# Borx25/CPU-Raytracing-experiments

Hardware: AMD Instinct MI355X
Metric: Mray/s (primary+bounce) (higher is better)
Workload: dtype f32; 1 GPU; cfg4: 4096x4096 px, S(100000) spheres + SAH BVH, MIS, Policy.max_bounces=9 (primary+8 bounces), 5 buckets, 64 accumulations/step; fixed image, tile rows split over the GPUs; image=4096x4096, spheres=100000, max_bounces=9, buckets=5, parallelism=single GPU, batches_in_flight=1, accumulations_per_batch=63, accumulations_per_batch_limit=63

## Files before the change

cpu-raytracing-experiments_amd/__init__.py:

```python
from __future__ import annotations

import ctypes as C
import os
import subprocess

import numpy as np

from . import distributed as distributed
from . import hdr as hdr
from . import scene as scene
from .scene import MATERIAL, NODE, SPHERE, Camera, Scene

_HERE = os.path.dirname(os.path.abspath(__file__))
CSRC = os.path.join(_HERE, "csrc")
LIB_PATH = os.path.join(CSRC, "libmirt.so")

MIRT_OK, MIRT_NOT_READY = 0, 1
AOV_DEPTH, AOV_NORMAL, AOV_ALBEDO = 0, 1, 2
AOV_PLANES = 7
KERNEL_CLASSES = ("raygen", "trace", "shade", "shadow", "resolve")


class MirtError(RuntimeError):
    pass
# ... 64 lines not shown
        "mirt_aov_floats": [P, C.POINTER(C.c_size_t)],
        "mirt_read_aov": [P, vp],
        "mirt_aov_device": [P, C.POINTER(vp), C.POINTER(C.c_size_t)],
        "mirt_load_aov": [P, vp, i32],
        "mirt_render_aov": [P, i32, vp],
        "mirt_get_counters": [P, C.POINTER(Counters)],
        "mirt_get_kernel_times": [P, C.POINTER(KernelTimes), i32],
        "mirt_get_stream": [P, C.POINTER(vp)],
        "mirt_debug_raygen": [P, u32, vp, vp],
        "mirt_debug_trace_closest": [P, C.c_size_t, vp, vp, vp, vp],
        "mirt_debug_trace_shadow": [P, C.c_size_t, vp, vp, vp, vp],
        "mirt_debug_math": [P, i32, C.c_size_t, vp, vp],
        "mirt_debug_info": [P, vp],
        "mirt_debug_tree": [P, vp, C.c_size_t, vp],
        "mirt_debug_primary_lists": [P, vp],
        "mirt_debug_allow_half_boxes": [P, i32],
    }
    G = C.c_void_p
    sigs.update({
        "mirt_group_create": [vp, i32, C.POINTER(G)],
        "mirt_group_destroy": [G],
        "mirt_group_size": [G, C.POINTER(i32)],
        "mirt_group_member": [G, i32, C.POINTER(P)],
        "mirt_group_set_scene": [G, vp, vp, u32, vp, u32, vp, u32, vp, u32, vp, vp, u32, u32],
        "mirt_group_set_camera": [G, vp, vp, f, f, f, f],
        "mirt_group_set_lens": [G, f, f],
        "mirt_group_pick_focus": [G, u32, u32, C.POINTER(f), C.POINTER(f)],
        "mirt_group_set_policy": [G, C.POINTER(Policy)],
        "mirt_group_set_gloss_decay": [G, vp, u32],
        "mirt_group_set_stream_order": [G, u32],
# ... 290 lines not shown
        return d

    def debug_tree(self):
        info = (C.c_uint32 * 4)()
        self._check(self._lib.mirt_debug_tree(self._ctx, None, 0, info))
        n, rec_bytes = int(info[0]), int(info[1])
        words = np.zeros((n, rec_bytes // 4), dtype=np.uint32)
        self._check(self._lib.mirt_debug_tree(self._ctx, _ptr(words), words.nbytes, info))
        return words, dict(zip(("records", "record_bytes", "layout", "depth"), [int(v) for v in info]))

    def debug_primary_lists(self) -> list:
        out = (C.c_uint32 * 10)()
        self._check(self._lib.mirt_debug_primary_lists(self._ctx, out))
        return [int(v) for v in out]

    def stream_handle(self) -> int:
        p = C.c_void_p()
        self._check(self._lib.mirt_get_stream(self._ctx, C.byref(p)))
        return p.value

    def debug_raygen(self, accumulations: int):
        n = (self.width // 16) * (self.height // 16) * 256
        p = np.empty((3, n), dtype=np.float32)
        d = np.empty((3, n), dtype=np.float32)
        self._check(self._lib.mirt_debug_raygen(self._ctx, accumulations, _ptr(p), _ptr(d)))
        return p, d

    def debug_trace_closest(self, p: np.ndarray, d: np.ndarray):
        p = np.ascontiguousarray(p, dtype=np.float32); d = np.ascontiguousarray(d, dtype=np.float32)
        n = p.shape[1]
# ... 189 lines not shown
```

cpu-raytracing-experiments_amd/csrc/kernels.hpp:

```cpp
#pragma once
#include <hip/hip_runtime.h>
#include <stdint.h>
#include "device_math.hpp"

namespace mirt {

constexpr uint32_t kBlock = 256;
constexpr uint32_t kShadeBlock = 512;
constexpr uint32_t kTraceBlock = 1024;
constexpr uint32_t kLdsStack = 16;
constexpr uint32_t kLdsStackWide = 12;
constexpr uint32_t kLeafBit = 0x80000000u;
constexpr uint32_t kTileSize = 256;
constexpr uint32_t kTileRoot = 16;
constexpr uint32_t kStack = 64;
constexpr uint32_t kDestAccum = 0x80000000u;

struct SceneDev {
	const float4* recs;
	const float4* spheres;
	const int32_t* prim_mat;
	const float4* light_sphere;
	const float4* light_emit;
	const float4* mat_albedo;
// ... 242 lines not shown
	float px, py, pz, dx, dy, dz;
	RaySlab rs;
	float tfar;
	int32_t prim;
	uint32_t cur, sp;
};
struct TravSpill { uint32_t e[kStack - kLdsStackWide]; };
constexpr float kAlphaFat = 0.03f;
MIRT_DI bool trav_begin(Trav& t, float px, float py, float pz, float dx, float dy, float dz, float tfar, float alpha_extra = 0.0f) {
	t.px = px; t.py = py; t.pz = pz; t.dx = dx; t.dy = dy; t.dz = dz;
	float alpha;
	t.rs = make_slab(px, py, pz, dx, dy, dz, alpha, alpha_extra);
	t.tfar = tfar; t.prim = -1; t.cur = 0; t.sp = 0;
	return alpha > kAlphaFat;
}
constexpr int kClosest = 0, kAnyHit = 1, kCollect = 2;
constexpr uint32_t kCandMax = 31, kCandStride = 32, kCandOverflow = 0xffffffffu;
struct Collect { uint32_t* cand; float rho; uint32_t n_pix; };
MIRT_DI void collect_leaf(bool on, float4 s, uint32_t prim, uint32_t pix, const Collect& col, Trav& t) {
	uint32_t cnt = static_cast<uint32_t>(t.prim);
	if (on & (cnt < kCandMax)) col.cand[static_cast<size_t>(1u + cnt) * col.n_pix + pix] = prim;
	cnt += on ? 1u : 0u;
	t.prim = static_cast<int32_t>(cnt);
	const f3 oc{ s.x - t.px, s.y - t.py, s.z - t.pz };
	const float oc2 = dot3(oc, oc), b = dot3(f3{ t.dx, t.dy, t.dz }, oc);
	const float len = __builtin_sqrtf(oc2);
	const float reach = __builtin_sqrtf(__builtin_fmaxf(oc2 - b * b, 0.0f)) + col.rho * len;
	const float slack = (s.w - reach * reach) - (0x1p-17f * oc2 + 1e-6f * s.w);
	const bool cover = on & (b > 0.0f) & (oc2 > s.w * 1.002f) & (slack > 0.0f);
	const float F = ((b + col.rho * len) - __builtin_sqrtf(__builtin_fmaxf(slack, 0.0f))) * 1.001f + 1e-4f;
	t.tfar = (cover & (F < t.tfar)) ? F : t.tfar;
}
typedef __attribute__((address_space(3))) int16_t lds_i16;
template <bool HALF, bool ST16>
MIRT_DI void stack_put(const TraceLds lds, TravSpill& spill, uint32_t sp, uint32_t ref) {
	constexpr uint32_t lds_entries = (HALF && !ST16) ? kLdsStackWide : kLdsStack;
// ... 109 lines not shown
		if (hd && (!cd || !d_cd)) { stack_put<true, ST16>(lds, spill, sp, r3); sp += 1u; }
	}
	uint32_t next = any ? near : kHalt;
	if (!any & (sp != 0u)) { --sp; next = stack_get<true, ST16>(lds, spill, sp); }
	t.sp = sp;
	t.cur = next;
}
template <int MODE, bool COUNT, bool ALL_LDS, bool HALF, bool ST16>
MIRT_DI void leaf_step(const SceneDev& sc, const TraceLds lds, Trav& t, TravSpill& spill, bool& occluded, uint32_t& n_spheres, uint32_t pix, const Collect& col) {
	const uint32_t first = t.cur & ~kLeafBit;
	float4 s;
	if (ALL_LDS) s = to_float4(lds.spheres[first]); else s = sc.spheres[first];
	if (COUNT) n_spheres += 1u;
	bool fin = false;
	if (MODE == kAnyHit) { occluded = sphere_occludes_sel(s, t.px, t.py, t.pz, t.dx, t.dy, t.dz, t.tfar); fin = occluded; }
	else if (MODE == kCollect) { collect_leaf(true, s, first, pix, col, t); fin = static_cast<uint32_t>(t.prim) > kCandMax; }
	else sphere_closest_sel(true, s, static_cast<int32_t>(first), t.px, t.py, t.pz, t.dx, t.dy, t.dz, t.tfar, t.prim);
	uint32_t sp = t.sp;
	t.cur = kHalt;
	if (!fin & (sp != 0u)) { --sp; t.cur = stack_get<HALF, ST16>(lds, spill, sp); }
	t.sp = sp;
}

constexpr uint32_t kChunkMax = 512;
constexpr uint32_t kLeafBatch = 16;
constexpr uint32_t kRefillIdle = 32;
constexpr uint32_t kNone = 0xffffffffu;
struct FatList { uint32_t* count; uint32_t* rays; uint32_t capacity; };
struct WaveWindow { uint32_t beg, end, chunk_end, offset, chunk; bool more; };
MIRT_DI uint32_t pick_chunk(uint32_t n, uint32_t chunk_max) {
	const uint32_t waves = gridDim.x * (blockDim.x >> 6);
// ... 30 lines not shown
                              LoadRay load_ray, StoreResult store_result, const Collect col = Collect{ nullptr, 0.0f, 0u }) {
	WaveWindow w{ 0, 0, 0, 0, pick_chunk(n, sc.chunk_max), true };
	Trav t;
	TravSpill spill;
	uint32_t ri = kNone;
	bool occluded = false;
	t.cur = kHalt;
	for (;;) {
		if ((ri != kNone) & (t.cur == kHalt)) { store_result(ri, t, occluded); ri = kNone; }
		{
			const uint32_t got = wave_take(ri == kNone, w, q, n, work_next);
			if (got != kNone) {
				float px, py, pz, dx, dy, dz, tf;
				load_ray(got, px, py, pz, dx, dy, dz, tf);
				ri = got; occluded = false;
				if (MODE == kCollect) {
					if (trav_begin(t, px, py, pz, dx, dy, dz, tf, col.rho)) { t.prim = static_cast<int32_t>(kCandMax + 1u); t.cur = kHalt; }
					else t.prim = 0;
				} else if (trav_begin(t, px, py, pz, dx, dy, dz, tf)) {
					const uint32_t k = atomicAdd(fat.count, 1u);
					if (k < fat.capacity) { fat.rays[k] = got; ri = kNone; t.cur = kHalt; }
				}
			}
		}
		const bool work_left = w.more || w.beg != w.chunk_end;
		if (__ballot(ri != kNone) == 0ull) { if (!work_left) break; continue; }
		const bool can_refill = work_left;
		for (;;) {
			const bool at_leaf = static_cast<int32_t>(t.cur) < 0, at_node = t.cur < kHalt;
			const unsigned long long leaf_m = __ballot(at_leaf), node_m = __ballot(at_node);
			const unsigned long long walking = leaf_m | node_m;
			if (walking == 0ull) break;
// ... 342 lines not shown
			float tfar = MIRT_FLT_MAX; int32_t prim = -1;
			for (uint32_t k = 0; k < kCandRegs; k++) if (id[k] >= 0) sphere_closest_tie(s[k], id[k], ox, oy, oz, d.x, d.y, d.z, tfar, prim);
			for (uint32_t k = kCandRegs; k < kCandMax; k++) {
				if (__ballot(k < cnt) == 0ull) break;
				if (k < cnt) {
					const uint32_t j = cand[static_cast<size_t>(k + 1u) * fp.n_pix + pix];
					sphere_closest_tie(sc.spheres[j], static_cast<int32_t>(j), ox, oy, oz, d.x, d.y, d.z, tfar, prim);
				}
			}
			if (COUNT) c_spheres += cnt;
			const size_t i = static_cast<size_t>(slot) * fp.n_pix + pix;
			hit_out[i] = HitRec{ tfar, prim };
		}
	}
	if (COUNT) wave_sum(c_spheres, &ctr->spheres);
}

constexpr uint32_t kAovPlanes = 7;
constexpr float kAovMissDepth = 1e4f;
template <bool LENS = false>
__global__ __launch_bounds__(kBlock) void k_first_hit_aov(SceneDev sc, FrameParams fp, const HitRec* __restrict__ hit_in, const float4* __restrict__ mat_colour, float* __restrict__ aov, LensParams lens) {
	f3 O{ fp.cam.pos[0], fp.cam.pos[1], fp.cam.pos[2] };
	for (uint32_t pix = blockIdx.x * kBlock + threadIdx.x; pix < fp.n_pix; pix += gridDim.x * kBlock) {
		uint32_t tile; int32_t x, y;
		pixel_xy(fp, pix, tile, x, y);
		const uint32_t seed = (tile * kTileSize + (pix & 255u)) * (fp.max_bounces * 2u + 1u);
		float* w = aov + static_cast<size_t>(pix >> 8) * (kAovPlanes * kTileSize) + (pix & 255u);
		float sum[kAovPlanes];
		for (uint32_t k = 0; k < kAovPlanes; k++) sum[k] = w[k * kTileSize];
		int32_t cached = -1;
// ... 660 lines not shown
```

cpu-raytracing-experiments_amd/csrc/mirt_capi.hip:

```cpp
#include "../../include/mirt.h"
#include "kernels.hpp"
#include "bvh_layout.hpp"
#include "bvh_build.hpp"
#include "lbvh_build.hpp"

#include <hip/hip_runtime.h>
#include <algorithm>
#include <cstdarg>
#include <cstdio>
#include <cstdlib>
#include <cstring>
#include <string>
#include <vector>

using namespace mirt;

namespace {

thread_local std::string g_create_error;

struct DeviceBuffer {
	void* ptr = nullptr;
	size_t bytes = 0;
	hipError_t ensure(size_t want) {
// ... 51 lines not shown
	DeviceBuffer recs, recs_wide, spheres, prim_mat, light_sphere, light_emit, mat_albedo, mat_emission, mat_ggx, hdri;
	SceneDev scene{};
	std::vector<float> gloss_decay;
	uint32_t stream_order = 0;
	DeviceBuffer gloss_decay_dev;
	bool gloss_decay_dev_valid = false;
	CameraParams camera{};
	LensParams lens{};
	uint32_t bvh_depth = 0;
	DeviceBuffer cand;
	DeviceBuffer cand_listed;
	DeviceBuffer cand_words;
	hipEvent_t cand_built = nullptr;
	uint64_t cand_gen = 0;
	bool cand_valid = false;
	bool allow_half = true;

	DeviceBuffer accumulator;
	uint32_t aov_on = 0;
	DeviceBuffer aov;
	hipEvent_t aov_prev = nullptr;
	DeviceBuffer framebuffer;
	float* frame_host = nullptr;
	size_t frame_host_bytes = 0;
	DeviceBuffer counters;
	std::vector<PipeSlot> slots;
	uint64_t planned_for = 0;
	uint32_t batch_mem_cap = 256;
	uint32_t capacity = 0;
	uint32_t seg_cap = 0;
// ... 85 lines not shown
struct BatchCounters {
	uint32_t* w; uint32_t nb, seg_cap;
	static size_t words(uint32_t nb) { return static_cast<size_t>(2 * nb + 2) * kQueueWords + static_cast<size_t>(nb) * 4 + 8; }
	Queue queue(uint32_t k) const { return Queue{ w + static_cast<size_t>(k) * kQueueWords, seg_cap }; }
	uint32_t* word(uint32_t k) const { return w + static_cast<size_t>(2 * nb + 2) * kQueueWords + k; }
	Queue stream_queue(uint32_t b) const { return queue(b); }
	Queue shadow_queue(uint32_t b) const { return queue(nb + 1 + b); }
	Queue empty_queue() const { return queue(2 * nb + 1); }
	uint32_t* closest_work(uint32_t b) const { return word(b); }
	uint32_t* shadow_work(uint32_t b) const { return word(nb + b); }
	FatList fat_closest(uint32_t b, uint32_t* lists) const { return FatList{ word(2 * nb + b), lists, kFatCapacity }; }
	FatList fat_shadow(uint32_t b, uint32_t* lists) const { return FatList{ word(3 * nb + b), lists + kFatCapacity, kFatCapacity }; }
};
struct CandWords {
	uint32_t* w;
	static constexpr size_t kWords = 4;
	uint32_t* work() const { return w; }
	uint32_t* unused_fat_count() const { return w + 1; }
	uint32_t* listed_pixels() const { return w + 2; }
};
BatchCounters batch_counters(const mirt_ctx* c, const PipeSlot& sl) { return BatchCounters{ sl.counts.as<uint32_t>(), c->policy.max_bounces, c->seg_cap }; }
uint32_t wanted_slots(const mirt_ctx* c) {
	if (c->policy.streams) return std::min<uint32_t>(c->policy.streams, 8u);
	return static_cast<uint64_t>(c->n_tiles) * kTileSize * batch_limit(c) >= kSerialRays ? 1u : 3u;
}
uint64_t streams_bytes(const mirt_ctx* c) {
	const uint64_t rays = static_cast<uint64_t>(c->n_tiles) * kTileSize * batch_limit(c);
	return wanted_slots(c) * (rays * 4u * kStreamPlanes + rays * 12u);
}

void plan_batches(mirt_ctx* c) {
	const uint64_t n_pix = static_cast<uint64_t>(c->n_tiles) * kTileSize;
	if (c->policy.max_batch || n_pix == 0 || c->planned_for == n_pix) return;
	c->batch_mem_cap = kMaxBatch;
// ... 165 lines not shown

const decltype(&k_trace<true, kPrimaryNone>) kTrace[2][3] = {
	{ k_trace<true, kPrimaryNone>, k_trace<true, kPrimaryAll>, k_trace<true, kPrimaryList> },
	{ k_trace<false, kPrimaryNone>, k_trace<false, kPrimaryAll>, k_trace<false, kPrimaryList> } };
const decltype(&k_trace_fat<true, kPrimaryNone>) kTraceFat[2][3] = {
	{ k_trace_fat<true, kPrimaryNone>, k_trace_fat<true, kPrimaryAll>, k_trace_fat<true, kPrimaryList> },
	{ k_trace_fat<false, kPrimaryNone>, k_trace_fat<false, kPrimaryAll>, k_trace_fat<false, kPrimaryList> } };
const decltype(&k_primary_cand<true>) kPrimaryCand[2] = { k_primary_cand<true>, k_primary_cand<false> };
const decltype(&k_primary_hits<true>) kPrimaryHits[2] = { k_primary_hits<true>, k_primary_hits<false> };
const decltype(&k_shade<false, false>) kShade[2][2] = { { k_shade<false, false>, k_shade<false, true> }, { k_shade<true, false>, k_shade<true, true> } };
const decltype(&k_tile_stream<false>) kTileStream[2] = { k_tile_stream<false>, k_tile_stream<true> };
static_assert(kPrimaryNone == 0 && kPrimaryAll == 1 && kPrimaryList == 2, "kTrace / kTraceFat are indexed by PRIMARY");
const decltype(&k_trace<true, kPrimaryNone>) kTraceLens[2] = { k_trace<true, kPrimaryAll, true>, k_trace<false, kPrimaryAll, true> };
const decltype(&k_trace_fat<true, kPrimaryNone>) kTraceFatLens[2] = { k_trace_fat<true, kPrimaryAll, true>, k_trace_fat<false, kPrimaryAll, true> };
const decltype(&k_shade<false, false>) kShadeLens[2] = { k_shade<true, false, true>, k_shade<true, true, true> };

struct TraceLaunch {
	StreamBuf in; HitRec* hit;
	Queue closest_queue; uint32_t* closest_work;
	ShadowBuf sh; ShadowSink sink;
	Queue shadow_queue; uint32_t* shadow_work;
	FatList fat_closest, fat_shadow;
	const uint32_t* listed_pixels;
	DevCounters* ctr;
};
void launch_trace(const mirt_ctx* c, hipStream_t st, const SceneDev& sc, const FrameParams& fp, uint64_t n_rays, bool count, int primary, const TraceLaunch& t, bool lens = false) {
	hipLaunchKernelGGL(lens ? kTraceLens[!count] : kTrace[!count][primary], dim3(trace_grid(c, n_rays)), dim3(kTraceBlock), trace_lds(c), st, sc, fp, t.in, t.hit, t.closest_queue, t.closest_work,
	                   t.sh, t.sink, t.shadow_queue, t.shadow_work, t.fat_closest, t.fat_shadow, t.ctr, c->lens);
	const uint32_t fat_grid = sc.n_spheres > 4096 ? static_cast<uint32_t>(c->n_cu) * 2u : 64u;
	if (sc.use_bvh) hipLaunchKernelGGL(lens ? kTraceFatLens[!count] : kTraceFat[!count][primary], dim3(fat_grid), dim3(1024), 0, st, sc, fp, t.in, t.hit, t.fat_closest, t.sh, t.sink, t.fat_shadow, t.ctr, t.listed_pixels, c->lens);
}

int launch_tile_stream(mirt_ctx* c, hipStream_t st, const SceneDev& sc, const FrameParams& fp, uint32_t batch_n, float* contrib, DevCounters* ctr, bool count) {
	if (!c->gloss_decay_dev_valid) {
		HIP_TRY(c, sync_all(c));
		HIP_TRY(c, c->gloss_decay_dev.ensure(std::max<size_t>(c->gloss_decay.size(), 1) * sizeof(float)));
		if (!c->gloss_decay.empty()) HIP_TRY(c, hipMemcpy(c->gloss_decay_dev.ptr, c->gloss_decay.data(), c->gloss_decay.size() * sizeof(float), hipMemcpyHostToDevice));
		c->gloss_decay_dev_valid = true;
	}
	Bracket t(c, MIRT_K_TRACE, st);
	hipLaunchKernelGGL(kTileStream[c->policy.brdf != 0], dim3(c->n_tiles * batch_n), dim3(kTileSize), 0, st, sc, fp, contrib, ctr, c->mat_ggx.as<float4>(),
	                   c->gloss_decay_dev.as<float>(), static_cast<uint32_t>(c->gloss_decay.size()), count ? 1u : 0u);
	return MIRT_OK;
}

int build_primary_lists(mirt_ctx* c, const SceneDev& sc, const FrameParams& fp, bool count) {
	HIP_TRY(c, c->cand.ensure(static_cast<size_t>(fp.n_pix) * kCandStride * sizeof(uint32_t)));
	HIP_TRY(c, c->cand_listed.ensure(static_cast<size_t>(fp.n_pix) * sizeof(uint32_t)));
	HIP_TRY(c, c->cand_words.ensure(CandWords::kWords * sizeof(uint32_t)));
	if (!c->cand_built) HIP_TRY(c, hipEventCreateWithFlags(&c->cand_built, hipEventDisableTiming));
	const CandWords cw{ c->cand_words.as<uint32_t>() };
	HIP_TRY(c, hipMemsetAsync(cw.w, 0, CandWords::kWords * sizeof(uint32_t), c->stream));
	{ Bracket t(c, MIRT_K_TRACE);
	  const FatList none{ cw.unused_fat_count(), nullptr, 0u };
	  hipLaunchKernelGGL(kPrimaryCand[!count], dim3(trace_grid(c, fp.n_pix)), dim3(kTraceBlock), trace_lds(c), c->stream, sc, fp, c->cand.as<uint32_t>(), bundle_half_angle(c),
	                     cw.work(), none, c->counters.as<DevCounters>(), c->cand_listed.as<uint32_t>(), cw.listed_pixels()); }
	HIP_TRY(c, hipGetLastError());
	HIP_TRY(c, hipEventRecord(c->cand_built, c->stream));
	c->cand_gen++;
	c->cand_valid = true;
	return MIRT_OK;
}

int launch_first_hit_aov(mirt_ctx* c, PipeSlot& sl, hipStream_t st, const SceneDev& sc, const FrameParams& fp) {
	const bool pipelined = c->slots.size() > 1;
	if (pipelined) {
		if (!sl.aov_done) HIP_TRY(c, hipEventCreateWithFlags(&sl.aov_done, hipEventDisableTiming));
		if (c->aov_prev && c->aov_prev != sl.aov_done) HIP_TRY(c, hipStreamWaitEvent(st, c->aov_prev, 0));
	}
	{ Bracket t(c, MIRT_K_RESOLVE, st);
	  const uint32_t grid = static_cast<uint32_t>(std::min<uint64_t>((static_cast<uint64_t>(fp.n_pix) + kBlock - 1) / kBlock, static_cast<uint64_t>(c->n_cu) * 64u));
	  hipLaunchKernelGGL(lens_on(c) ? k_first_hit_aov<true> : k_first_hit_aov<false>, dim3(grid), dim3(kBlock), 0, st, sc, fp, sl.hit, c->policy.brdf ? c->mat_ggx.as<float4>() : c->scene.mat_albedo,
// ... 21 lines not shown
	const SceneDev sc = trace_scene(c);
	const bool count = c->policy.count_traffic != 0;
	const uint32_t sgrid = static_cast<uint32_t>(std::min<uint64_t>((total + kShadeBlock - 1) / kShadeBlock, static_cast<uint64_t>(c->n_cu) * c->tune_shade_wgs));
	{
		const uint64_t n_chunks = (static_cast<uint64_t>(fp.n_pix) + kShadeBlock - 1) / kShadeBlock;
		const uint64_t want = (8ull * sgrid + n_chunks - 1) / n_chunks;
		fp.first_groups = static_cast<uint32_t>(std::min<uint64_t>(std::max<uint64_t>(want, 1), batch_n));
	}

	if (pipelined && sl.in_use) HIP_TRY(c, hipStreamWaitEvent(st, sl.merged, 0));
	if (c->debug_poison_contrib)
		HIP_TRY(c, hipMemsetD32Async(reinterpret_cast<hipDeviceptr_t>(sl.contrib.ptr), 0x7fc0deadu, sl.contrib.bytes / sizeof(float), st));
	HIP_TRY(c, hipMemsetAsync(bc.w, 0, BatchCounters::words(nb) * sizeof(uint32_t), st));
	if (bundle) {
		if (!c->cand_valid || count) { const int r = build_primary_lists(c, sc, fp, count); if (r) return r; }
		if (pipelined && sl.cand_gen != c->cand_gen) { HIP_TRY(c, hipStreamWaitEvent(st, c->cand_built, 0)); sl.cand_gen = c->cand_gen; }
	}
	const CandWords cw{ c->cand_words.as<uint32_t>() };
	if (c->stream_order) {
		const int r = launch_tile_stream(c, st, sc, fp, batch_n, contrib, ctr, count);
		if (r) return r;
	} else {
		for (uint32_t bounce = 0; bounce < nb; bounce++) {
			const StreamBuf& in = sl.stream_buf[bounce & 1u];
			const StreamBuf& out = sl.stream_buf[(bounce & 1u) ^ 1u];
			const bool shadow_pending = fp.mis && bounce > 0;
			const bool lists = bounce == 0 && bundle;
			{ Bracket t(c, MIRT_K_TRACE, st);
			  if (lists) {
			    const uint32_t hgrid = static_cast<uint32_t>(std::min<uint64_t>((static_cast<uint64_t>(fp.n_pix) + kBlock - 1) / kBlock, static_cast<uint64_t>(c->n_cu) * 64u));
			    hipLaunchKernelGGL(kPrimaryHits[!count], dim3(hgrid), dim3(kBlock), 0, st, sc, fp, c->cand.as<uint32_t>(), sl.hit, ctr);
			  }
			  const ShadowSink sink{ in.path, in.px, in.py, in.pz, contrib, batch_n, fp.pix_bits, nullptr };
			  StreamBuf rays = in;
			  if (lists) rays.path = c->cand_listed.as<uint32_t>();
			  const TraceLaunch tl{ rays, sl.hit, lists ? Queue{ cw.listed_pixels(), 0u } : bc.stream_queue(bounce), bc.closest_work(bounce),
			                        sl.shadow_buf, sink, shadow_pending ? bc.shadow_queue(bounce - 1) : bc.empty_queue(), bc.shadow_work(shadow_pending ? bounce - 1 : 0),
			                        bc.fat_closest(bounce, fat_lists), bc.fat_shadow(bounce, fat_lists), lists ? cw.listed_pixels() : nullptr, ctr };
			  launch_trace(c, st, sc, fp, total, count, lists ? kPrimaryList : bounce == 0 ? kPrimaryAll : kPrimaryNone, tl, bounce == 0 && lens); }
			if (bounce == 0 && c->aov_on) { const int r = launch_first_hit_aov(c, sl, st, sc, fp); if (r) return r; }
			{ Bracket t(c, MIRT_K_SHADE, st);
			  const float decay = bounce < c->gloss_decay.size() ? c->gloss_decay[bounce] : 0.0f;
			  hipLaunchKernelGGL(bounce == 0 && lens ? kShadeLens[c->policy.brdf != 0] : kShade[bounce == 0][c->policy.brdf != 0], dim3(sgrid), dim3(kShadeBlock), 0, st, sc, fp, in, sl.hit, out, sl.shadow_buf, bounce,
			                     bc.stream_queue(bounce), bc.stream_queue(bounce + 1), bc.shadow_queue(bounce), contrib, ctr, mat_ggx, decay, c->lens); }
		}
	}
	HIP_TRY(c, hipGetLastError());
	if (pipelined) {
		HIP_TRY(c, hipEventRecord(sl.batch_done, st));
		HIP_TRY(c, hipStreamWaitEvent(c->stream, sl.batch_done, 0));
	}
	{ Bracket t(c, MIRT_K_RESOLVE);
	  hipLaunchKernelGGL(k_merge_contrib, dim3(grid_for(c, static_cast<uint64_t>(c->n_tiles) * (kTileSize / 4u))), dim3(kBlock), 0, c->stream,
	                     c->accumulator.as<float4>(), sl.contrib.as<float4>(), c->n_tiles, c->policy.buckets, batch_n, fp.acc_base); }
// ... 138 lines not shown
	if (!why.empty()) return fail(c, MIRT_ERR_ARG, "%s BVH rejected: %s", caller_tree ? "caller's" : "internal", why.c_str());
	t.n_recs = static_cast<uint32_t>(t.f32.size() / 16);
	t.is_half = c->allow_half && mirt_host::build_half_records(t.f32, t.half);
	uint32_t wide_levels = 0;
	t.is_wide = t.is_half && c->tune_wide && mirt_host::build_wide_half_records(t.f32, t.wide, &wide_levels);
	if (t.is_wide) t.n_recs = static_cast<uint32_t>(t.wide.size() / 16);
	return t.is_wide ? upload(c, c->recs, t.wide) : t.is_half ? upload(c, c->recs, t.half) : upload(c, c->recs, t.f32);
}

int plan_trace_lds(mirt_ctx* c) {
	const LdsPlan p = lds_plan(c);
	c->scene.stack16 = p.stack16; c->scene.lds_recs = p.lds_recs; c->scene.lds_spheres = p.lds_spheres;
	const int lds_max = static_cast<int>(kLdsPerCu);
	for (const auto& row : kTrace) for (const auto k : row) HIP_TRY(c, hipFuncSetAttribute(reinterpret_cast<const void*>(k), hipFuncAttributeMaxDynamicSharedMemorySize, lds_max));
	for (const auto k : kPrimaryCand) HIP_TRY(c, hipFuncSetAttribute(reinterpret_cast<const void*>(k), hipFuncAttributeMaxDynamicSharedMemorySize, lds_max));
	for (const auto k : kTraceLens) HIP_TRY(c, hipFuncSetAttribute(reinterpret_cast<const void*>(k), hipFuncAttributeMaxDynamicSharedMemorySize, lds_max));
	return MIRT_OK;
}

void commit_scene(mirt_ctx* c, const SceneArgs& a, const SceneRecords& t) {
	SceneDev& s = c->scene;
	s.recs = t.in_recs_wide ? c->recs_wide.as<float4>() : c->recs.as<float4>(); s.spheres = c->spheres.as<float4>(); s.prim_mat = c->prim_mat.as<int32_t>();
	s.light_sphere = c->light_sphere.as<float4>(); s.light_emit = c->light_emit.as<float4>();
	s.mat_albedo = c->mat_albedo.as<float4>(); s.mat_emission = c->mat_emission.as<float4>();
	s.hdri = c->hdri.as<float4>();
	s.n_spheres = a.n_spheres; s.n_recs = t.n_recs; s.n_mat = a.n_materials; s.n_lights = a.n_lights;
	s.half_boxes = t.is_half ? 1u : 0u;
	s.wide = t.is_wide ? 1u : 0u;
	c->bvh_depth = t.depth;
	for (int k = 0; k < 3; k++) s.ambient[k] = a.ambient_color[k];
// ... 48 lines not shown
	int n = 0;
	hipError_t e = hipGetDeviceCount(&n);
	if (e != hipSuccess || n <= 0) return fail(nullptr, MIRT_ERR_NO_DEVICE, "no HIP device available (%s); mirt has no CPU path", hipGetErrorString(e));
	if (device < 0 || device >= n) return fail(nullptr, MIRT_ERR_ARG, "device %d out of range (have %d)", device, n);
	e = hipSetDevice(device);
	if (e != hipSuccess) return fail(nullptr, MIRT_ERR_HIP, "hipSetDevice: %s", hipGetErrorString(e));
	mirt_ctx* c = new mirt_ctx();
	c->device = device;
	if (const char* e = std::getenv("MIRT_TUNE_CHUNK")) c->tune_chunk = static_cast<uint32_t>(std::min(std::max(std::atoi(e), 64), 65536)) & ~63u;
	if (const char* e = std::getenv("MIRT_TUNE_REFILL_IDLE")) c->tune_refill_idle = static_cast<uint32_t>(std::min(std::max(std::atoi(e), 1), 64));
	if (const char* e = std::getenv("MIRT_TUNE_WIDE")) c->tune_wide = std::atoi(e) != 0 ? 1u : 0u;
	if (const char* e = std::getenv("MIRT_TUNE_LEAF_BATCH")) c->tune_leaf_batch = static_cast<uint32_t>(std::min(std::max(std::atoi(e), 1), 64));
	if (const char* e = std::getenv("MIRT_TUNE_TRACE_WGS")) c->tune_trace_wgs = std::atoi(e) == 1 ? 1u : 2u;
	if (const char* e = std::getenv("MIRT_TUNE_SHADE_WGS")) c->tune_shade_wgs = static_cast<uint32_t>(std::min(std::max(std::atoi(e), 1), 16));
	if (const char* e = std::getenv("MIRT_DEBUG_POISON_CONTRIB")) c->debug_poison_contrib = std::atoi(e) != 0;
	hipDeviceProp_t prop;
	if (hipGetDeviceProperties(&prop, device) == hipSuccess) c->n_cu = prop.multiProcessorCount > 0 ? prop.multiProcessorCount : 256;
	e = hipStreamCreateWithFlags(&c->stream, hipStreamNonBlocking);
	if (e == hipSuccess) e = c->counters.ensure(sizeof(DevCounters));
	if (e == hipSuccess) e = hipMemsetAsync(c->counters.ptr, 0, sizeof(DevCounters), c->stream);
	if (e != hipSuccess) { int r = fail(nullptr, MIRT_ERR_HIP, "context setup: %s", hipGetErrorString(e)); delete c; return r; }
	*out = c;
	return MIRT_OK;
}

int mirt_destroy(mirt_ctx* c) {
	if (!c) return MIRT_ERR_ARG;
	(void)hipSetDevice(c->device);
	(void)sync_all(c);
	harvest(c);
	for (PipeSlot& sl : c->slots) {
		sl.arena.release(); sl.counts.release(); sl.contrib.release(); sl.fat.release();
		if (sl.batch_done) (void)hipEventDestroy(sl.batch_done);
		if (sl.merged) (void)hipEventDestroy(sl.merged);
		if (sl.aov_done) (void)hipEventDestroy(sl.aov_done);
		if (sl.stream) (void)hipStreamDestroy(sl.stream);
	}
	c->slots.clear();
	for (hipEvent_t e : c->free_events) (void)hipEventDestroy(e);
	DeviceBuffer* bufs[] = { &c->recs, &c->recs_wide, &c->spheres, &c->prim_mat, &c->light_sphere, &c->light_emit, &c->mat_albedo, &c->mat_emission,
	                         &c->mat_ggx, &c->hdri, &c->accumulator, &c->aov, &c->framebuffer, &c->counters, &c->gloss_decay_dev,
	                         &c->cand, &c->cand_listed, &c->cand_words };
	for (DeviceBuffer* b : bufs) b->release();
	if (c->frame_host) (void)hipHostFree(c->frame_host);
	if (c->cand_built) (void)hipEventDestroy(c->cand_built);
	if (c->stream) (void)hipStreamDestroy(c->stream);
	delete c;
	return MIRT_OK;
}

int mirt_set_scene(mirt_ctx* c, const mirt_sphere* geometry, const mirt_sphere* bvh_prims, uint32_t n_spheres,
                   const mirt_bvh_node* nodes, uint32_t n_nodes, const mirt_material* materials, uint32_t n_materials,
                   const int32_t* lights, uint32_t n_lights, const float ambient_color[3],
                   const float* hdri_rgba, uint32_t hdri_w, uint32_t hdri_h) {
	if (!c) return MIRT_ERR_ARG;
	{ const int fr = flush_deferred(c); if (fr) return fr; }
	const SceneArgs a{ geometry, bvh_prims, n_spheres, nodes, n_nodes, materials, n_materials, lights, n_lights, ambient_color, hdri_rgba, hdri_w, hdri_h };
// ... 424 lines not shown
	if (!c->policy.use_bvh || c->scene.n_recs == 0 || c->n_tiles == 0) return fail(c, MIRT_ERR_STATE, "needs policy.use_bvh, a tree and at least one tile");
	{ const int fr = flush_deferred(c); if (fr) return fr; }
	HIP_TRY(c, hipSetDevice(c->device));
	if ((r = ensure_streams(c))) return r;
	HIP_TRY(c, sync_all(c));
	const FrameParams fp = frame_params(c, 0, 1);
	if (!c->cand_valid && (r = build_primary_lists(c, trace_scene(c), fp, false))) return r;
	std::vector<uint32_t> host(static_cast<size_t>(fp.n_pix));
	HIP_TRY(c, hipMemcpyAsync(host.data(), c->cand.ptr, host.size() * 4, hipMemcpyDeviceToHost, c->stream));
	HIP_TRY(c, hipStreamSynchronize(c->stream));
	for (int k = 0; k < 10; k++) hist[k] = 0;
	for (size_t p = 0; p < fp.n_pix; p++) { const uint32_t n = host[p]; hist[n == kCandOverflow ? 9 : std::min<uint32_t>(n, 8u)]++; }
	return MIRT_OK;
}

int mirt_debug_info(mirt_ctx* c, uint32_t out[8]) {
	if (!c || !out) return MIRT_ERR_ARG;
	const SceneDev& s = c->scene;
	const LdsPlan p = lds_plan(c);
	out[0] = s.n_recs; out[1] = s.lds_recs; out[2] = s.lds_spheres; out[3] = c->bvh_depth; out[4] = s.half_boxes | (s.wide << 1);
	out[5] = p.launch_bytes; out[6] = p.wgs_per_cu; out[7] = static_cast<uint32_t>(c->n_cu);
	return MIRT_OK;
}
int mirt_debug_tree(mirt_ctx* c, void* dst, size_t capacity_bytes, uint32_t info[4]) {
	if (!c) return MIRT_ERR_ARG;
	if (!info) return fail(c, MIRT_ERR_ARG, "debug_tree: info is NULL");
	if (!c->have_scene) return fail(c, MIRT_ERR_STATE, "mirt_set_scene has not been called");
	const SceneDev& s = c->scene;
	const uint32_t rec_bytes = (s.half_boxes && !s.wide) ? 32u : 64u;
	info[0] = s.n_recs; info[1] = rec_bytes; info[2] = s.wide ? 2u : s.half_boxes ? 1u : 0u; info[3] = c->bvh_depth;
// ... 13 lines not shown
```

include/mirt.h:

```cpp
#ifndef MIRT_H
#define MIRT_H

#include <stddef.h>
#include <stdint.h>

#ifdef __cplusplus
extern "C" {
#endif

#define MIRT_OK              0
#define MIRT_NOT_READY       1
#define MIRT_ERR_ARG        -1
#define MIRT_ERR_HIP        -2
#define MIRT_ERR_STATE      -3
#define MIRT_ERR_NO_DEVICE  -4

#define MIRT_TILE_ROOT     16u
#define MIRT_TILE_SIZE    256u
#define MIRT_MAX_MATERIALS 63u
#define MIRT_MAX_BUCKETS   16u
#define MIRT_BVH_STACK     64u

typedef struct mirt_sphere {
	float   position[3];
// ... 144 lines not shown
int mirt_group_read_accumulator(mirt_group* group, float* host_dst);
int mirt_group_render(mirt_group* group, float* rgba_host);
int mirt_group_set_aov(mirt_group* group, uint32_t on);
int mirt_group_aov_floats(const mirt_group* group, size_t* n_floats);
int mirt_group_read_aov(mirt_group* group, float* host_dst);
int mirt_group_render_aov(mirt_group* group, int which, float* out);
int mirt_group_rccl_selftest(int device, size_t n_floats);

int mirt_debug_raygen(mirt_ctx* ctx, uint32_t accumulations, float* p_xyz, float* dir_xyz);
int mirt_debug_trace_closest(mirt_ctx* ctx, size_t n, const float* p_xyz, const float* dir_xyz, float* tfar_out, int32_t* primID_out);
int mirt_debug_trace_shadow(mirt_ctx* ctx, size_t n, const float* p_xyz, const float* dir_xyz, const float* tfar, uint8_t* occluded_out);
int mirt_debug_math(mirt_ctx* ctx, int fn, size_t n, const float* in, float* out);
int mirt_debug_info(mirt_ctx* ctx, uint32_t out[8]);
int mirt_debug_tree(mirt_ctx* ctx, void* dst, size_t capacity_bytes, uint32_t info[4]);
int mirt_debug_primary_lists(mirt_ctx* ctx, uint32_t hist[10]);
int mirt_debug_allow_half_boxes(mirt_ctx* ctx, int allow);

#ifdef __cplusplus
}
#endif
#endif
```

Baseline: 9496 Mray/s.

## Add second-tier primary candidate lists for pixels overflowing the first-tier cap

Pixels whose primary-ray candidate sphere lists overflowed the 31-entry cap used to fall back to full BVH traversal for every sample. A second collection pass now builds lists of up to 127 candidates for those pixels, provided they are at most a quarter of all pixels. A new hits kernel tests each sample against its list, and only the remaining residual pixels are traced through the BVH. This costs extra memory, a one-off build with host syncs, and another kernel launch per batch.

```diff
diff --git a/cpu-raytracing-experiments_amd/__init__.py b/cpu-raytracing-experiments_amd/__init__.py
--- a/cpu-raytracing-experiments_amd/__init__.py
+++ b/cpu-raytracing-experiments_amd/__init__.py
@@ -102,6 +102,7 @@
         "mirt_debug_info": [P, vp],
         "mirt_debug_tree": [P, vp, C.c_size_t, vp],
         "mirt_debug_primary_lists": [P, vp],
+        "mirt_debug_overflow_lists": [P, vp],
         "mirt_debug_allow_half_boxes": [P, i32],
     }
     G = C.c_void_p
@@ -422,6 +423,12 @@
         self._check(self._lib.mirt_debug_primary_lists(self._ctx, out))
         return [int(v) for v in out]
 
+    def debug_overflow_lists(self) -> dict:
+        out = (C.c_uint32 * 20)()
+        self._check(self._lib.mirt_debug_overflow_lists(self._ctx, out))
+        v = [int(x) for x in out]
+        return {"overflow": v[0], "second_tier": v[1], "residual": v[2], "cap": v[3], "hist8": v[4:]}
+
     def stream_handle(self) -> int:
         p = C.c_void_p()
         self._check(self._lib.mirt_get_stream(self._ctx, C.byref(p)))
diff --git a/cpu-raytracing-experiments_amd/csrc/kernels.hpp b/cpu-raytracing-experiments_amd/csrc/kernels.hpp
--- a/cpu-raytracing-experiments_amd/csrc/kernels.hpp
+++ b/cpu-raytracing-experiments_amd/csrc/kernels.hpp
@@ -280,12 +280,15 @@
 	t.tfar = tfar; t.prim = -1; t.cur = 0; t.sp = 0;
 	return alpha > kAlphaFat;
 }
-constexpr int kClosest = 0, kAnyHit = 1, kCollect = 2;
+constexpr int kClosest = 0, kAnyHit = 1, kCollect = 2, kCollect2 = 3;
 constexpr uint32_t kCandMax = 31, kCandStride = 32, kCandOverflow = 0xffffffffu;
-struct Collect { uint32_t* cand; float rho; uint32_t n_pix; };
+constexpr uint32_t kCand2Max = 127;
+struct Collect { uint32_t* cand; float rho; uint32_t n_pix; uint32_t cap = kCandMax; };
+template <int MODE> MIRT_DI uint32_t collect_cap(const Collect& col) { return MODE == kCollect2 ? col.cap : kCandMax; }
+template <int MODE>
 MIRT_DI void collect_leaf(bool on, float4 s, uint32_t prim, uint32_t pix, const Collect& col, Trav& t) {
 	uint32_t cnt = static_cast<uint32_t>(t.prim);
-	if (on & (cnt < kCandMax)) col.cand[static_cast<size_t>(1u + cnt) * col.n_pix + pix] = prim;
+	if (on & (cnt < collect_cap<MODE>(col))) col.cand[static_cast<size_t>(1u + cnt) * col.n_pix + pix] = prim;
 	cnt += on ? 1u : 0u;
 	t.prim = static_cast<int32_t>(cnt);
 	const f3 oc{ s.x - t.px, s.y - t.py, s.z - t.pz };
@@ -425,7 +428,7 @@
 	if (COUNT) n_spheres += 1u;
 	bool fin = false;
 	if (MODE == kAnyHit) { occluded = sphere_occludes_sel(s, t.px, t.py, t.pz, t.dx, t.dy, t.dz, t.tfar); fin = occluded; }
-	else if (MODE == kCollect) { collect_leaf(true, s, first, pix, col, t); fin = static_cast<uint32_t>(t.prim) > kCandMax; }
+	else if (MODE == kCollect || MODE == kCollect2) { collect_leaf<MODE>(true, s, first, pix, col, t); fin = static_cast<uint32_t>(t.prim) > collect_cap<MODE>(col); }
 	else sphere_closest_sel(true, s, static_cast<int32_t>(first), t.px, t.py, t.pz, t.dx, t.dy, t.dz, t.tfar, t.prim);
 	uint32_t sp = t.sp;
 	t.cur = kHalt;
@@ -486,8 +489,8 @@
 				float px, py, pz, dx, dy, dz, tf;
 				load_ray(got, px, py, pz, dx, dy, dz, tf);
 				ri = got; occluded = false;
-				if (MODE == kCollect) {
-					if (trav_begin(t, px, py, pz, dx, dy, dz, tf, col.rho)) { t.prim = static_cast<int32_t>(kCandMax + 1u); t.cur = kHalt; }
+				if (MODE == kCollect || MODE == kCollect2) {
+					if (trav_begin(t, px, py, pz, dx, dy, dz, tf, col.rho)) { t.prim = static_cast<int32_t>(collect_cap<MODE>(col) + 1u); t.cur = kHalt; }
 					else t.prim = 0;
 				} else if (trav_begin(t, px, py, pz, dx, dy, dz, tf)) {
 					const uint32_t k = atomicAdd(fat.count, 1u);
@@ -860,6 +863,64 @@
 		}
 	}
 	if (COUNT) wave_sum(c_spheres, &ctr->spheres);
+}
+template <bool LATE>
+__global__ __launch_bounds__(kTraceBlock, 8) void k_primary_cand2(SceneDev sc, FrameParams fp, uint32_t* __restrict__ cand2, float rho, uint32_t cap, uint32_t* work, FatList unused,
+                                                                 const uint32_t* __restrict__ ov_pix, uint32_t n_ov, uint32_t* __restrict__ res_pix, uint32_t* __restrict__ res_count) {
+	extern __shared__ float4 lds[];
+	if (n_ov == 0 || static_cast<uint64_t>(blockIdx.x) * 64u >= n_ov) return;
+	const TraceLds tl = stage_bvh(sc, lds);
+	uint32_t c_nodes = 0, c_spheres = 0;
+	auto load_ray = [&](uint32_t j, float& px, float& py, float& pz, float& dx, float& dy, float& dz, float& tf) {
+		uint32_t tile; int32_t x, y;
+		pixel_xy(fp, ov_pix[j], tile, x, y);
+		const f3 d = camera_ray_dir(fp.cam, x, y, 0.5f, 0.5f);
+		px = fp.cam.pos[0]; py = fp.cam.pos[1]; pz = fp.cam.pos[2]; dx = d.x; dy = d.y; dz = d.z; tf = MIRT_FLT_MAX;
+	};
+	auto store_result = [&](uint32_t j, const Trav& t, bool) {
+		const bool over = static_cast<uint32_t>(t.prim) > cap;
+		cand2[j] = over ? kCandOverflow : static_cast<uint32_t>(t.prim);
+		const unsigned long long m = __ballot(over);
+		if (over) {
+			const uint32_t leader = static_cast<uint32_t>(__ffsll(static_cast<long long>(m))) - 1u;
+			uint32_t first = 0;
+			if (lane_id() == leader) first = atomicAdd(res_count, static_cast<uint32_t>(__popcll(m)));
+			first = __builtin_amdgcn_readlane(first, leader);
+			res_pix[first + mask_rank(m)] = ov_pix[j];
+		}
+	};
+	trace_queue<kCollect2, false>(sc, tl, Queue{ nullptr, 0u }, n_ov, work, unused, c_nodes, c_spheres, load_ray, store_result, Collect{ cand2, rho, n_ov, cap });
+}
+constexpr uint32_t kHits2Unroll = 4;
+template <bool LATE>
+__global__ __launch_bounds__(kBlock) void k_primary_hits2(SceneDev sc, FrameParams fp, const uint32_t* __restrict__ cand2, const uint32_t* __restrict__ ov_pix, uint32_t n_ov,
+                                                         HitRec* __restrict__ hit_out) {
+	const uint32_t lane = threadIdx.x & 63u, n_waves = gridDim.x * (kBlock >> 6);
+	const float ox = fp.cam.pos[0], oy = fp.cam.pos[1], oz = fp.cam.pos[2];
+	for (uint32_t j = __builtin_amdgcn_readfirstlane(blockIdx.x * (kBlock >> 6) + (threadIdx.x >> 6)); j < n_ov; j += n_waves) {
+		const uint32_t cnt = cand2[j];
+		if (cnt == kCandOverflow) continue;
+		const uint32_t pix = ov_pix[j];
+		uint32_t tile; int32_t x, y;
+		pixel_xy(fp, pix, tile, x, y);
+		const uint32_t seed = (tile * kTileSize + (pix & 255u)) * (fp.max_bounces * 2u + 1u);
+		const uint32_t* __restrict__ list = cand2 + n_ov + j;
+		for (uint32_t base = 0; base < fp.batch_n; base += 64u) {
+			const uint32_t slot = base + lane;
+			uint32_t rng = hash_2d(fp.acc_base + slot + 1u, seed);
+			const float s0 = rand_unit_float(rng);
+			const float s1 = rand_unit_float(rng);
+			const f3 d = camera_ray_dir(fp.cam, x, y, s0, s1);
+			float tfar = MIRT_FLT_MAX; int32_t prim = -1;
+			for (uint32_t k = 0; k < cnt; k += kHits2Unroll) {
+				uint32_t id[kHits2Unroll]; float4 s[kHits2Unroll];
+				for (uint32_t u = 0; u < kHits2Unroll; u++) id[u] = list[static_cast<size_t>(min(k + u, cnt - 1u)) * n_ov];
+				for (uint32_t u = 0; u < kHits2Unroll; u++) s[u] = sc.spheres[id[u]];
+				for (uint32_t u = 0; u < kHits2Unroll; u++) sphere_closest_tie(s[u], static_cast<int32_t>(id[u]), ox, oy, oz, d.x, d.y, d.z, tfar, prim);
+			}
+			if (slot < fp.batch_n) hit_out[static_cast<size_t>(slot) * fp.n_pix + pix] = HitRec{ tfar, prim };
+		}
+	}
 }
 
 constexpr uint32_t kAovPlanes = 7;
diff --git a/cpu-raytracing-experiments_amd/csrc/mirt_capi.hip b/cpu-raytracing-experiments_amd/csrc/mirt_capi.hip
--- a/cpu-raytracing-experiments_amd/csrc/mirt_capi.hip
+++ b/cpu-raytracing-experiments_amd/csrc/mirt_capi.hip
@@ -89,6 +89,13 @@
 	hipEvent_t cand_built = nullptr;
 	uint64_t cand_gen = 0;
 	bool cand_valid = false;
+	DeviceBuffer cand2;
+	DeviceBuffer cand2_residual;
+	uint32_t cand2_n_ov = 0;
+	uint32_t cand2_n_residual = 0;
+	bool cand2_built = false;
+	bool cand2_in_use = false;
+	uint32_t cand2_cap = kCand2Max;
 	bool allow_half = true;
 
 	DeviceBuffer accumulator;
@@ -204,10 +211,12 @@
 };
 struct CandWords {
 	uint32_t* w;
-	static constexpr size_t kWords = 4;
+	static constexpr size_t kWords = 8;
 	uint32_t* work() const { return w; }
 	uint32_t* unused_fat_count() const { return w + 1; }
 	uint32_t* listed_pixels() const { return w + 2; }
+	uint32_t* work2() const { return w + 3; }
+	uint32_t* residual_pixels() const { return w + 4; }
 };
 BatchCounters batch_counters(const mirt_ctx* c, const PipeSlot& sl) { return BatchCounters{ sl.counts.as<uint32_t>(), c->policy.max_bounces, c->seg_cap }; }
 uint32_t wanted_slots(const mirt_ctx* c) {
@@ -403,6 +412,8 @@
 const decltype(&k_trace<true, kPrimaryNone>) kTraceLens[2] = { k_trace<true, kPrimaryAll, true>, k_trace<false, kPrimaryAll, true> };
 const decltype(&k_trace_fat<true, kPrimaryNone>) kTraceFatLens[2] = { k_trace_fat<true, kPrimaryAll, true>, k_trace_fat<false, kPrimaryAll, true> };
 const decltype(&k_shade<false, false>) kShadeLens[2] = { k_shade<true, false, true>, k_shade<true, true, true> };
+const decltype(&k_primary_cand2<true>) kPrimaryCand2 = k_primary_cand2<true>;
+const decltype(&k_primary_hits2<true>) kPrimaryHits2 = k_primary_hits2<true>;
 
 struct TraceLaunch {
 	StreamBuf in; HitRec* hit;
@@ -433,6 +444,35 @@
 	return MIRT_OK;
 }
 
+constexpr uint32_t kCand2Share = 4;
+int build_secondary_lists(mirt_ctx* c, const SceneDev& sc, const FrameParams& fp) {
+	const CandWords cw{ c->cand_words.as<uint32_t>() };
+	c->cand2_in_use = false; c->cand2_n_ov = c->cand2_n_residual = 0;
+	HIP_TRY(c, hipMemsetAsync(cw.work2(), 0, 2 * sizeof(uint32_t), c->stream));
+	HIP_TRY(c, hipMemcpyAsync(&c->cand2_n_ov, cw.listed_pixels(), sizeof(uint32_t), hipMemcpyDeviceToHost, c->stream));
+	HIP_TRY(c, hipStreamSynchronize(c->stream));
+	const uint32_t n_ov = c->cand2_n_ov;
+	if (n_ov > fp.n_pix) return fail(c, MIRT_ERR_STATE, "candidate lists: %u of %u pixels listed", n_ov, fp.n_pix);
+	c->cand2_built = true;
+	if (n_ov == 0) { c->cand2_in_use = true; return MIRT_OK; }
+	if (n_ov > fp.n_pix / kCand2Share) { c->cand2_n_residual = n_ov; return MIRT_OK; }
+	if (c->cand2.ensure(static_cast<size_t>(n_ov) * (c->cand2_cap + 1u) * sizeof(uint32_t)) != hipSuccess ||
+	    c->cand2_residual.ensure(static_cast<size_t>(n_ov) * sizeof(uint32_t)) != hipSuccess) {
+		(void)hipGetLastError();
+		c->cand2.release(); c->cand2_residual.release(); c->cand2_n_residual = n_ov;
+		return MIRT_OK;
+	}
+	const FatList none{ cw.unused_fat_count(), nullptr, 0u };
+	hipLaunchKernelGGL(kPrimaryCand2, dim3(trace_grid(c, n_ov)), dim3(kTraceBlock), trace_lds(c), c->stream, sc, fp, c->cand2.as<uint32_t>(), bundle_half_angle(c), c->cand2_cap,
+	                   cw.work2(), none, c->cand_listed.as<uint32_t>(), n_ov, c->cand2_residual.as<uint32_t>(), cw.residual_pixels());
+	HIP_TRY(c, hipGetLastError());
+	HIP_TRY(c, hipMemcpyAsync(&c->cand2_n_residual, cw.residual_pixels(), sizeof(uint32_t), hipMemcpyDeviceToHost, c->stream));
+	HIP_TRY(c, hipStreamSynchronize(c->stream));
+	if (c->cand2_n_residual > n_ov) return fail(c, MIRT_ERR_STATE, "candidate lists: %u of %u listed pixels left over", c->cand2_n_residual, n_ov);
+	c->cand2_in_use = true;
+	return MIRT_OK;
+}
+
 int build_primary_lists(mirt_ctx* c, const SceneDev& sc, const FrameParams& fp, bool count) {
 	HIP_TRY(c, c->cand.ensure(static_cast<size_t>(fp.n_pix) * kCandStride * sizeof(uint32_t)));
 	HIP_TRY(c, c->cand_listed.ensure(static_cast<size_t>(fp.n_pix) * sizeof(uint32_t)));
@@ -443,8 +483,10 @@
 	{ Bracket t(c, MIRT_K_TRACE);
 	  const FatList none{ cw.unused_fat_count(), nullptr, 0u };
 	  hipLaunchKernelGGL(kPrimaryCand[!count], dim3(trace_grid(c, fp.n_pix)), dim3(kTraceBlock), trace_lds(c), c->stream, sc, fp, c->cand.as<uint32_t>(), bundle_half_angle(c),
-	                     cw.work(), none, c->counters.as<DevCounters>(), c->cand_listed.as<uint32_t>(), cw.listed_pixels()); }
-	HIP_TRY(c, hipGetLastError());
+	                     cw.work(), none, c->counters.as<DevCounters>(), c->cand_listed.as<uint32_t>(), cw.listed_pixels());
+	  HIP_TRY(c, hipGetLastError()); }
+	c->cand2_built = c->cand2_in_use = false; c->cand2_n_ov = c->cand2_n_residual = 0;
+	if (!count) { const int r = build_secondary_lists(c, sc, fp); if (r) return r; }
 	HIP_TRY(c, hipEventRecord(c->cand_built, c->stream));
 	c->cand_gen++;
 	c->cand_valid = true;
@@ -496,6 +538,10 @@
 	HIP_TRY(c, hipMemsetAsync(bc.w, 0, BatchCounters::words(nb) * sizeof(uint32_t), st));
 	if (bundle) {
 		if (!c->cand_valid || count) { const int r = build_primary_lists(c, sc, fp, count); if (r) return r; }
+		else if (!c->cand2_built) {
+			const int r = build_secondary_lists(c, sc, fp); if (r) return r;
+			HIP_TRY(c, hipEventRecord(c->cand_built, c->stream)); c->cand_gen++;
+		}
 		if (pipelined && sl.cand_gen != c->cand_gen) { HIP_TRY(c, hipStreamWaitEvent(st, c->cand_built, 0)); sl.cand_gen = c->cand_gen; }
 	}
 	const CandWords cw{ c->cand_words.as<uint32_t>() };
@@ -508,18 +554,26 @@
 			const StreamBuf& out = sl.stream_buf[(bounce & 1u) ^ 1u];
 			const bool shadow_pending = fp.mis && bounce > 0;
 			const bool lists = bounce == 0 && bundle;
+			const bool tier2 = lists && !count && c->cand2_in_use;
 			{ Bracket t(c, MIRT_K_TRACE, st);
 			  if (lists) {
 			    const uint32_t hgrid = static_cast<uint32_t>(std::min<uint64_t>((static_cast<uint64_t>(fp.n_pix) + kBlock - 1) / kBlock, static_cast<uint64_t>(c->n_cu) * 64u));
 			    hipLaunchKernelGGL(kPrimaryHits[!count], dim3(hgrid), dim3(kBlock), 0, st, sc, fp, c->cand.as<uint32_t>(), sl.hit, ctr);
+			    if (tier2 && c->cand2_n_ov > c->cand2_n_residual) {
+			      const uint32_t h2grid = static_cast<uint32_t>(std::min<uint64_t>((static_cast<uint64_t>(c->cand2_n_ov) + kBlock / 64u - 1) / (kBlock / 64u), static_cast<uint64_t>(c->n_cu) * 64u));
+			      hipLaunchKernelGGL(kPrimaryHits2, dim3(h2grid), dim3(kBlock), 0, st, sc, fp, c->cand2.as<uint32_t>(), c->cand_listed.as<uint32_t>(), c->cand2_n_ov, sl.hit);
+			    }
 			  }
 			  const ShadowSink sink{ in.path, in.px, in.py, in.pz, contrib, batch_n, fp.pix_bits, nullptr };
 			  StreamBuf rays = in;
-			  if (lists) rays.path = c->cand_listed.as<uint32_t>();
-			  const TraceLaunch tl{ rays, sl.hit, lists ? Queue{ cw.listed_pixels(), 0u } : bc.stream_queue(bounce), bc.closest_work(bounce),
+			  uint32_t* const traced_count = tier2 ? cw.residual_pixels() : cw.listed_pixels();
+			  const uint64_t n_traced = tier2 ? static_cast<uint64_t>(c->cand2_n_residual) * batch_n : total;
+			  if (lists) rays.path = tier2 ? c->cand2_residual.as<uint32_t>() : c->cand_listed.as<uint32_t>();
+			  const TraceLaunch tl{ rays, sl.hit, lists ? Queue{ traced_count, 0u } : bc.stream_queue(bounce), bc.closest_work(bounce),
 			                        sl.shadow_buf, sink, shadow_pending ? bc.shadow_queue(bounce - 1) : bc.empty_queue(), bc.shadow_work(shadow_pending ? bounce - 1 : 0),
-			                        bc.fat_closest(bounce, fat_lists), bc.fat_shadow(bounce, fat_lists), lists ? cw.listed_pixels() : nullptr, ctr };
-			  launch_trace(c, st, sc, fp, total, count, lists ? kPrimaryList : bounce == 0 ? kPrimaryAll : kPrimaryNone, tl, bounce == 0 && lens); }
+			                        bc.fat_closest(bounce, fat_lists), bc.fat_shadow(bounce, fat_lists), lists ? traced_count : nullptr, ctr };
+			  if (!tier2 || n_traced)
+			    launch_trace(c, st, sc, fp, n_traced, count, lists ? kPrimaryList : bounce == 0 ? kPrimaryAll : kPrimaryNone, tl, bounce == 0 && lens); }
 			if (bounce == 0 && c->aov_on) { const int r = launch_first_hit_aov(c, sl, st, sc, fp); if (r) return r; }
 			{ Bracket t(c, MIRT_K_SHADE, st);
 			  const float decay = bounce < c->gloss_decay.size() ? c->gloss_decay[bounce] : 0.0f;
@@ -688,6 +742,7 @@
 	const int lds_max = static_cast<int>(kLdsPerCu);
 	for (const auto& row : kTrace) for (const auto k : row) HIP_TRY(c, hipFuncSetAttribute(reinterpret_cast<const void*>(k), hipFuncAttributeMaxDynamicSharedMemorySize, lds_max));
 	for (const auto k : kPrimaryCand) HIP_TRY(c, hipFuncSetAttribute(reinterpret_cast<const void*>(k), hipFuncAttributeMaxDynamicSharedMemorySize, lds_max));
+	HIP_TRY(c, hipFuncSetAttribute(reinterpret_cast<const void*>(kPrimaryCand2), hipFuncAttributeMaxDynamicSharedMemorySize, lds_max));
 	for (const auto k : kTraceLens) HIP_TRY(c, hipFuncSetAttribute(reinterpret_cast<const void*>(k), hipFuncAttributeMaxDynamicSharedMemorySize, lds_max));
 	return MIRT_OK;
 }
@@ -766,6 +821,7 @@
 	if (const char* e = std::getenv("MIRT_TUNE_TRACE_WGS")) c->tune_trace_wgs = std::atoi(e) == 1 ? 1u : 2u;
 	if (const char* e = std::getenv("MIRT_TUNE_SHADE_WGS")) c->tune_shade_wgs = static_cast<uint32_t>(std::min(std::max(std::atoi(e), 1), 16));
 	if (const char* e = std::getenv("MIRT_DEBUG_POISON_CONTRIB")) c->debug_poison_contrib = std::atoi(e) != 0;
+	if (const char* e = std::getenv("MIRT_DEBUG_CAND2_MAX")) c->cand2_cap = static_cast<uint32_t>(std::min(std::max(std::atoi(e), static_cast<int>(kCandMax) + 1), static_cast<int>(kCand2Max)));
 	hipDeviceProp_t prop;
 	if (hipGetDeviceProperties(&prop, device) == hipSuccess) c->n_cu = prop.multiProcessorCount > 0 ? prop.multiProcessorCount : 256;
 	e = hipStreamCreateWithFlags(&c->stream, hipStreamNonBlocking);
@@ -792,7 +848,7 @@
 	for (hipEvent_t e : c->free_events) (void)hipEventDestroy(e);
 	DeviceBuffer* bufs[] = { &c->recs, &c->recs_wide, &c->spheres, &c->prim_mat, &c->light_sphere, &c->light_emit, &c->mat_albedo, &c->mat_emission,
 	                         &c->mat_ggx, &c->hdri, &c->accumulator, &c->aov, &c->framebuffer, &c->counters, &c->gloss_decay_dev,
-	                         &c->cand, &c->cand_listed, &c->cand_words };
+	                         &c->cand, &c->cand_listed, &c->cand_words, &c->cand2, &c->cand2_residual };
 	for (DeviceBuffer* b : bufs) b->release();
 	if (c->frame_host) (void)hipHostFree(c->frame_host);
 	if (c->cand_built) (void)hipEventDestroy(c->cand_built);
@@ -1247,6 +1303,30 @@
 	return MIRT_OK;
 }
 
+int mirt_debug_overflow_lists(mirt_ctx* c, uint32_t out[20]) {
+	int r = check_ready(c); if (r) return r;
+	if (!out) return fail(c, MIRT_ERR_ARG, "out is NULL");
+	if (!c->policy.use_bvh || c->scene.n_recs == 0 || c->n_tiles == 0) return fail(c, MIRT_ERR_STATE, "needs policy.use_bvh, a tree and at least one tile");
+	{ const int fr = flush_deferred(c); if (fr) return fr; }
+	HIP_TRY(c, hipSetDevice(c->device));
+	if ((r = ensure_streams(c))) return r;
+	HIP_TRY(c, sync_all(c));
+	const FrameParams fp = frame_params(c, 0, 1);
+	if (!c->cand_valid && (r = build_primary_lists(c, trace_scene(c), fp, false))) return r;
+	if (!c->cand2_built) {
+		if ((r = build_secondary_lists(c, trace_scene(c), fp))) return r;
+		HIP_TRY(c, hipEventRecord(c->cand_built, c->stream)); c->cand_gen++;
+	}
+	for (int k = 0; k < 20; k++) out[k] = 0;
+	out[0] = c->cand2_n_ov; out[1] = c->cand2_n_ov - c->cand2_n_residual; out[2] = c->cand2_n_residual; out[3] = c->cand2_cap;
+	if (c->cand2_n_ov == 0 || c->cand2_n_residual == c->cand2_n_ov) return MIRT_OK;
+	std::vector<uint32_t> host(c->cand2_n_ov);
+	HIP_TRY(c, hipMemcpyAsync(host.data(), c->cand2.ptr, host.size() * 4, hipMemcpyDeviceToHost, c->stream));
+	HIP_TRY(c, hipStreamSynchronize(c->stream));
+	for (const uint32_t n : host) if (n != kCandOverflow) out[4 + std::min<uint32_t>(n / 8u, 15u)]++;
+	return MIRT_OK;
+}
+
 int mirt_debug_info(mirt_ctx* c, uint32_t out[8]) {
 	if (!c || !out) return MIRT_ERR_ARG;
 	const SceneDev& s = c->scene;
diff --git a/include/mirt.h b/include/mirt.h
--- a/include/mirt.h
+++ b/include/mirt.h
@@ -182,6 +182,7 @@
 int mirt_debug_info(mirt_ctx* ctx, uint32_t out[8]);
 int mirt_debug_tree(mirt_ctx* ctx, void* dst, size_t capacity_bytes, uint32_t info[4]);
 int mirt_debug_primary_lists(mirt_ctx* ctx, uint32_t hist[10]);
+int mirt_debug_overflow_lists(mirt_ctx* ctx, uint32_t out[20]);
 int mirt_debug_allow_half_boxes(mirt_ctx* ctx, int allow);
 
 #ifdef __cplusplus
```

After: 9607 Mray/s, median of 6. 1.2% higher.
